# do-mpc/do-mpc

Measured on AMD Instinct MI355X. Metric: MPC steps/sec (make_step wall-time), industrial_poly robust multi-stage, higher is better.
Workload: dtype f64

## Files before the change

__graft_entry__.py:

```python
import os
import subprocess
import sys

ROOT = os.path.dirname(os.path.abspath(__file__))
if ROOT not in sys.path:
    sys.path.insert(0, ROOT)

PREBUILT = [
    ("oscillating_masses", {}),
    ("batch_reactor", {}),
    ("batch_reactor", {"n_horizon": 50}),
    ("CSTR", {}),
    ("CSTR", {"n_robust": 0, "collocation_deg": 3}),
    ("CSTR", {"track_sign": -3000.0}),
    ("industrial_poly", {}),
    ("industrial_poly", {"n_robust": 2, "uncertainty": "paired"}),
    ("industrial_poly", {"collocation_deg": 3, "collocation_ni": 2, "n_horizon": 6}),
    ("kinematic_bicycle", {}),
    ("dynamic_bicycle", {}),
    ("kite", {"n_horizon": 20}),
    ("rotating_masses", {}),
    ("CSTR", {"custom_rterm": "default_as_expression"}),
    ("CSTR", {"custom_rterm": "custom"}),
    ("oscillating_masses", {"custom_rterm": "custom"}),
    ("oscillating_masses_dae", {}),
    ("dip", {}),
    ("CSTR", {"n_robust": 0, "nl_cons_check_colloc_points": True}),
    ("dip", {"n_horizon": 40, "nl_cons_check_colloc_points": True}),
    ("CSTR", {"nl_cons_single_slack": True}),
    ("CSTR", {"nl_cons_single_slack": True, "n_robust": 2, "n_horizon": 8, "uncertainty": {"alpha": [1.0, 1.05, 0.95], "beta": [1.0]}}),
    ("CSTR", {"nl_cons_single_slack": True, "n_robust": 0, "nl_cons_check_colloc_points": True}),
    ("CSTR", {"open_loop": True, "uncertainty": {"alpha": [1.0, 1.05, 0.95], "beta": [1.0]}}),
    ("CSTR", {"open_loop": True, "n_robust": 2, "n_horizon": 6, "uncertainty": {"alpha": [1.0, 1.05], "beta": [1.0]}, "soft_T_R": False}),
    ("shape_family:s1", {}), ("shape_family:s2", {}), ("shape_family:s3", {}), ("shape_family:s4", {}), ("shape_family:s5", {}),
    ("shape_family:s6", {}), ("shape_family:s7", {}), ("shape_family:s8", {}), ("shape_family:s9", {}),
]

PREBUILT_BATCH = [
    ("industrial_poly", {}), ("industrial_poly", {"n_robust": 2, "uncertainty": "paired"}),
    ("oscillating_masses", {}), ("CSTR", {}), ("CSTR", {"n_robust": 0, "collocation_deg": 3}), ("batch_reactor", {}), ("batch_reactor", {"n_horizon": 50}),
    ("rotating_masses", {}),
]
PREBUILT_BATCH_MHE = [("rotating_masses", "build_mhe", {}, {}), ("rotating_masses", "build_mhe_w", {"process_noise": True}, {}),
                      ("rotating_masses", "build_mhe_w", {"process_noise": True}, {"scaling": "MHE_W_SCALING"})]


PREBUILT_DEFS = [("CSTR", {}, "DOMPC_FORCE_DENSE=1"), ("batch_reactor", {}, "DOMPC_FORCE_DENSE=1"),
                 ("CSTR", {}, "DOMPC_GJ_U=1e9"), ("industrial_poly", {}, "DOMPC_GJ_U=1e9"),
                 ("batch_reactor", {}, "DOMPC_REG_GJ=0"), ("batch_reactor", {}, "DOMPC_GJ_U=1e9"),
                 ("industrial_poly", {}, "DOMPC_QUAD=0"), ("CSTR", {}, "DOMPC_QUAD=0"), ("CSTR", {"n_horizon": 5, "n_robust": 0}, "DOMPC_QUAD=0")]

PREBUILT_NODE_PACK = [("industrial_poly", {}), ("CSTR", {})] + [("shape_family:s%d" % i, {}) for i in range(1, 10)]
PREBUILT_BATCH_FAMILY = [("shape_family:s%d" % i, {}) for i in range(1, 10)]

PREBUILT_QUAD_LDS = [("DOMPC_QUAD_LDS=1", [("industrial_poly", {}), ("CSTR", {})]),
                     ("DOMPC_GJ_U=1e9", [("industrial_poly", {})]),
                     ("DOMPC_GJ_U=1e9 DOMPC_QUAD_LDS=1", [("industrial_poly", {})])]

PREBUILT_FWD_STAGE = [("DOMPC_FWD_STAGE=0", [("industrial_poly", {}), ("CSTR", {})]),
                      ("DOMPC_GJ_U=1e9 DOMPC_FWD_STAGE=0", [("industrial_poly", {})])]

PREBUILT_MO_READS = [("DOMPC_MO_BRANCHED=1", [("industrial_poly", {}), ("CSTR", {})]),
                     ("DOMPC_GJ_U=1e9 DOMPC_MO_BRANCHED=1", [("industrial_poly", {})])]

PREBUILT_SHARD = [
    ("CSTR", {}),
    ("industrial_poly", {"n_robust": 2, "uncertainty": "paired"}),
]


PREBUILT_MHE = [("rotating_masses", "build_mhe", {}, {}), ("rotating_masses", "build_mhe_w", {"process_noise": True}, {}),
                ("rotating_masses", "build_mhe_w", {"process_noise": True}, {"scaling": "MHE_W_SCALING"}),
                ("rotating_masses", "build_mhe", {"dae": True}, {}), ("rotating_masses", "build_mhe_w", {"process_noise": True, "dae": True}, {}),
                ("oscillating_masses", "build_mhe", {"estimation": True}, {}), ("oscillating_masses", "build_mhe", {"estimation": True, "dae": True}, {}),
                ("rotating_masses", "build_mhe_w", {"process_noise": True}, {"soft_limit": (-0.1, 0.01)}),
                ("rotating_masses", "build_mhe_w", {"process_noise": True}, {"soft_limit": (-0.1, 0.01), "nl_cons_single_slack": True}),
                ("rotating_masses", "build_mhe_w", {"process_noise": True, "input_meas_noise": False}, {})]


PREBUILT_ROUTE = [("oscillating_masses", "docstring", False, False), ("oscillating_masses", "tree", False, False),
                  ("industrial_poly", "tree", False, True), ("CSTR", "tree", False, True), ("batch_reactor", "tree", False, False),
                  ("oscillating_masses_dae", "tree", False, False), ("rotating_masses", "tree", False, False),
                  ("CSTR", "docstring", False, False), ("batch_reactor", "docstring", False, False), ("industrial_poly", "docstring", False, False),
                  ("oscillating_masses", None, True, False), ("CSTR", None, True, False), ("CSTR", "tree", True, False),
                  ("industrial_poly", None, True, False), ("industrial_poly", "tree", True, False), ("batch_reactor", None, True, False),
                  ("rotating_masses", None, True, False)]


def lowered_route_cases():
    from do_mpc_amd import controller
    from do_mpc_amd.examples import CASES
    tests = os.path.join(ROOT, "tests")
    if tests not in sys.path:
        sys.path.insert(0, tests)
    import route_cases as rc
    out = []
    orig = controller.HipIpmSolver
    controller.HipIpmSolver = _NoSolver
    try:
        for name, cost, rows, batch in PREBUILT_ROUTE:
            ex = CASES[name]
            mpc = rc.stopped_before_setup(lambda n: ex.build_mpc(ex.build_model()), name)
            mpc.prepare_nlp()
            if rows:
                rc.rows_at_three_nodes(mpc, name)
            if cost:
                rc.ADDED_COST[cost](mpc)
            mpc.create_nlp()
            out.append((f"{name} + {cost or ''}{' + rows' if rows else ''} (low-level route)", {}, mpc.generated_header, mpc.model_hash, batch))
    finally:
        controller.HipIpmSolver = orig
    return out


PREBUILT_PLANTS = ["oscillating_masses", "batch_reactor", "CSTR", "industrial_poly", "oscillating_masses_dae", "dip", "rotating_masses",
                   "triple_tank", "batch_reactor_lqr_dae", "batch_reactor_lqr_dae:build_dae_model", "cstr_lqr", "oscillating_masses_lqr"]

PREBUILT_PLANT_FAMILY = ["ode", "dae", "discrete"]


def lowered_plant_family(entries=None):
    from do_mpc_amd.simulator import Simulator
    tests = os.path.join(ROOT, "tests")
    if tests not in sys.path:
        sys.path.insert(0, tests)
    import plant_family_common as pf
    out = []
    for kind in (PREBUILT_PLANT_FAMILY if entries is None else entries):
        hdr = Simulator(pf.build_model(kind))._lower()
        out.append((kind, hdr, hdr.rsplit('PLANT_MODEL_HASH "', 1)[1].split('"')[0]))
    return out


PREBUILT_EKF = [("triple_tank", {}), ("oscillating_masses", {"estimation": True}), ("rotating_masses", {}), ("CSTR", {})]


def lowered_ekf(entries=None):
    from do_mpc_amd.ekf import EKF
    from do_mpc_amd.examples import CASES
    out = []
    for name, kw in (PREBUILT_EKF if entries is None else entries):
        hdr = EKF(CASES[name].build_model(**kw))._lower()
        out.append((name, kw, hdr, hdr.rsplit('EKF_MODEL_HASH "', 1)[1].split('"')[0]))
    return out


PREBUILT_EKF_DAE = ["masses", "nonlinear_discrete", "continuous", "dip", "batch_reactor", "limit", "status", "oscillating_masses_dae",
# ... 92 lines not shown
        if plant.startswith("family:"):
            (_, ph, p_hash), = lowered_plant_family([plant.split(":", 1)[1]])
        else:
            case, _, builder = plant.partition(":")
            ph = Simulator(getattr(CASES[case], builder or "build_model")())._lower()
            p_hash = ph.rsplit('PLANT_MODEL_HASH "', 1)[1].split('"')[0]
        (net_label, nh, n_hash), = lowered_ampc([shape])
        out.append((f"{plant} x {net_label}", ph, nh, p_hash, n_hash))
    return out


PREBUILT_ASMPC = [(1, 1), (4, 1), (4, 2), (17, 3), (3, 16), (64, 16)]


def lowered_asmpc(entries=None):
    from do_mpc_amd import lowering
    out = []
    for nx, nu in (PREBUILT_ASMPC if entries is None else entries):
        hdr = lowering.lower_asmpc(nx, nu)
        out.append((f"n_x = {nx}, n_u = {nu}", hdr, hdr.rsplit('ASMPC_MODEL_HASH "', 1)[1].split('"')[0]))
    return out


class _NoSolver:

    def __init__(self, *a, **k):
        pass


def lowered_models(which=None):
    from do_mpc_amd import controller
    from do_mpc_amd.examples import CASES
    out = []
    orig = controller.HipIpmSolver
    controller.HipIpmSolver = _NoSolver
    try:
        for name, kw in (PREBUILT if which is None else which):
            ex = CASES[name]
            mpc = ex.build_mpc(ex.build_model(), **kw)
            out.append((name, kw, mpc.generated_header, mpc.model_hash))
        if which is None:
            out += _lower_mhe(PREBUILT_MHE)
    finally:
        controller.HipIpmSolver = orig
    return out


def _lower_mhe(entries):
    from do_mpc_amd.examples import CASES
    out = []
    for name, builder, mkw, bkw in entries:
        ex = CASES[name]
        bkw = {k: (getattr(ex, v) if isinstance(v, str) else v) for k, v in bkw.items()}
        mhe = getattr(ex, builder)(ex.build_model(**mkw), **bkw)
        out.append((f"{name} ({builder})", {**mkw, **{k: "..." for k in bkw}}, mhe._mpc.generated_header, mhe._mpc.model_hash))
    return out


def lowered_mhe(entries):
    from do_mpc_amd import controller
    orig = controller.HipIpmSolver
    controller.HipIpmSolver = _NoSolver
    try:
        return _lower_mhe(entries)
    finally:
        controller.HipIpmSolver = orig


def build() -> None:
    from do_mpc_amd import build as nb
    import do_mpc_amd
    from concurrent.futures import ThreadPoolExecutor
    lib = nb.runtime_library()
    print("[build] runtime:", lib, flush=True)
    jobs = [(f"{name} {kw}", header, h, False, False, "") for name, kw, header, h in lowered_models()]
    jobs += [(f"{name} {kw}", header, h, True, False, "") for name, kw, header, h in lowered_models(PREBUILT_SHARD)]
    jobs += [(f"{name} {kw}", header, h, False, True, "") for name, kw, header, h in lowered_models(PREBUILT_BATCH + PREBUILT_BATCH_FAMILY)]
    jobs += [(f"{name} {kw}", header, h, False, True, "") for name, kw, header, h in lowered_mhe(PREBUILT_BATCH_MHE)]
    route = lowered_route_cases()
    jobs += [(f"{name} {kw}", header, h, False, False, "") for name, kw, header, h, _ in route]
    jobs += [(f"{name} {kw}", header, h, False, True, "") for name, kw, header, h, batch in route if batch]
    for name, kw, defs in PREBUILT_DEFS:
        jobs += [(f"{name} {kw}", header, h, False, False, defs) for _, _, header, h in lowered_models([(name, kw)])]
    for defs, classes in [("DOMPC_NODE_PACK=0", PREBUILT_NODE_PACK)] + PREBUILT_QUAD_LDS + PREBUILT_FWD_STAGE + PREBUILT_MO_READS:
        jobs += [(f"{name} {kw}", header, h, False, batch, defs) for name, kw, header, h in lowered_models(classes) for batch in (False, True)]
    with ThreadPoolExecutor(max_workers=max(1, min(len(jobs), (os.cpu_count() or 2) - 1))) as pool:
        outs = list(pool.map(lambda j: nb.model_code_object(j[1], j[2], shard=j[3], batch_only=j[4], defs=j[5]), jobs))
    for (label, _, _, shard, batch, defs), co in zip(jobs, outs):
        print(f"[build] {label}{' [' + defs + ']' if defs else ''}{' (tree sharding)' if shard else ''}{' (batch only)' if batch else ''}: {co}", flush=True)
    from do_mpc_amd.examples import CASES
    from do_mpc_amd.simulator import Simulator
    for name in PREBUILT_PLANTS:
        case, _, builder = name.partition(":")
        hdr = Simulator(getattr(CASES[case], builder or "build_model")())._lower()
        co = nb.plant_code_object(hdr, hdr.rsplit('PLANT_MODEL_HASH "', 1)[1].split('"')[0])
        print(f"[build] plant {name}: {co}")
    for kind, hdr, h in lowered_plant_family():
        print(f"[build] plant of the probe family '{kind}': {nb.plant_code_object(hdr, h)}")
    failed = []
    for entry in PREBUILT_EKF:
        try:
            for name, kw, hdr, h in lowered_ekf([entry]):
                print(f"[build] filter {name} {kw}: {nb.ekf_code_object(hdr, h)}")
        except Exception as e:
            failed.append(entry)
            print(f"[build] filter {entry[0]} {entry[1]}: FAILED\n{e}")
    for entry in PREBUILT_EKF_DAE:
        try:
            for name, hdr, h in lowered_ekf_dae([entry]):
                print(f"[build] filter of a model with algebraic states '{name}': {nb.ekf_code_object(hdr, h)}")
        except Exception as e:
            failed.append(entry)
            print(f"[build] filter of a model with algebraic states '{entry}': FAILED\n{e}")
    failed_lqr = []
    for entry in PREBUILT_LQR:
        try:
            for label, hdr, h in lowered_lqr([entry]):
                print(f"[build] LQR design {label}: {nb.lqr_code_object(hdr, h)}")
        except Exception as e:
            failed_lqr.append(entry)
            print(f"[build] LQR design {entry}: FAILED\n{e}")
    failed_ampc = []
    for entry in PREBUILT_AMPC:
        try:
            for label, hdr, h in lowered_ampc([entry]):
                print(f"[build] approximate MPC network {label}: {nb.ampc_code_object(hdr, h)}")
        except Exception as e:
            failed_ampc.append(entry)
            print(f"[build] approximate MPC network {entry}: FAILED\n{e}")
    failed_ampc_loop = []
    for entry in PREBUILT_AMPC_LOOP:
        try:
            for label, ph, nh, p_hash, n_hash in lowered_ampc_loop([entry]):
                co = nb.ampc_loop_code_object(ph, nh, nb.ampc_loop_pair_hash(p_hash, n_hash))
                print(f"[build] approximate MPC loop {label}: {co}")
                if entry[1] not in PREBUILT_AMPC:
                    print(f"[build] approximate MPC network of that pair: {nb.ampc_code_object(nh, n_hash)}")
        except Exception as e:
            failed_ampc_loop.append(entry)
            print(f"[build] approximate MPC loop {entry}: FAILED\n{e}")
    failed_asmpc = []
    for entry in PREBUILT_ASMPC:
        try:
            for label, hdr, h in lowered_asmpc([entry]):
                print(f"[build] sensitivity-based MPC law {label}: {nb.asmpc_code_object(hdr, h)}")
        except Exception as e:
            failed_asmpc.append(entry)
            print(f"[build] sensitivity-based MPC law {entry}: FAILED\n{e}")
    mk = os.path.join(ROOT, "oracle", "Makefile")
    if os.path.exists(mk):
        subprocess.run(["make", "-C", os.path.join(ROOT, "oracle")], check=True)
    if failed:
        raise RuntimeError(f"extended Kalman filter code objects that could not be built: {failed}")
    if failed_lqr:
        raise RuntimeError(f"LQR design code objects that could not be built: {failed_lqr}")
    if failed_ampc:
        raise RuntimeError(f"approximate MPC code objects that could not be built: {failed_ampc}")
    if failed_ampc_loop:
        raise RuntimeError(f"approximate MPC loop code objects that could not be built: {failed_ampc_loop}")
    if failed_asmpc:
        raise RuntimeError(f"sensitivity-based MPC law code objects that could not be built: {failed_asmpc}")


def smoke() -> None:
    import numpy as np
    from do_mpc_amd.examples import CASES
    from oracle import ipm
# ... 64 lines not shown
```

do_mpc_amd/csrc/dompc_kernel.h:

```cpp
#pragma once
#include <math.h>
#include <stdint.h>
#include "dompc_kargs.h"
#include "dompc_lanes.h"

namespace dompc {

#ifndef DOMPC_HOST_EMU
#define DOMPC_PHASE __device__ inline
#else
#define DOMPC_PHASE static inline
#endif

constexpr int NX = DOMPC_NX, NU = DOMPC_NU, NP = DOMPC_NP, NTVP = DOMPC_NTVP;
#ifndef DOMPC_EPS_GLOBAL
#define DOMPC_EPS_GLOBAL 0
#endif
constexpr bool EPS_GLOBAL = DOMPC_EPS_GLOBAL != 0 && DOMPC_NS > 0 && DOMPC_NE > 0;
constexpr int NS = EPS_GLOBAL ? 0 : DOMPC_NS;
constexpr int NSE = DOMPC_NS;
constexpr int NVG_MAX = 32;
constexpr int NZ = DOMPC_NZ;
constexpr int DEG = DOMPC_DEG, NI = DOMPC_NI, M = DOMPC_M;
#ifndef DOMPC_NL_COLLOC
#define DOMPC_NL_COLLOC 0
#endif
#ifndef DOMPC_FREE_ROOT
#define DOMPC_FREE_ROOT 0
#endif
#ifndef DOMPC_LT_END
#define DOMPC_LT_END 0
#endif
#ifndef DOMPC_NL_DUP
#define DOMPC_NL_DUP 0
#endif
#if !DOMPC_FREE_ROOT
DOMPC_FN double dompc_aterm_f(const double*, const double*, const double*, const double*) { return 0.0; }
DOMPC_FN void dompc_aterm(const double*, const double*, const double*, const double*, double*, double*, double*) {}
#endif
constexpr bool FREE_ROOT = DOMPC_FREE_ROOT != 0, LT_END = DOMPC_LT_END != 0 && M > 0;
constexpr int NEB = DOMPC_NE;
constexpr int NLP = (DOMPC_NL_COLLOC && M > 0) ? M : 1;
constexpr bool NL_DUP = DOMPC_NL_DUP != 0 && NEB > 0;
constexpr int NLB = NLP + (NL_DUP ? 1 : 0);
constexpr int NE = NEB * NLB;
constexpr bool NL_COLLOC = DOMPC_NL_COLLOC && M > 0 && NEB > 0;
DOMPC_HD constexpr int nl_pt(int blk) { return blk < NLP ? blk : NLP - 1; }
#ifndef DOMPC_FORCE_DENSE
#define DOMPC_FORCE_DENSE 0
#endif
constexpr bool DENSE_EDGE = DOMPC_NZ > 0 || NL_COLLOC || NL_DUP || LT_END || DOMPC_FORCE_DENSE;
DOMPC_HD inline int nl_slack(int i) { return DOMPC_NL_SLACK[NLB == 1 ? i : i % NEB]; }
constexpr int NA = NX + NU;
constexpr int NV = NU + NS;
constexpr int NYT = NA + NV;
constexpr int MZ = NZ > 0 ? (M > 0 ? M : 1) : 0;
constexpr int NWX = M * NX;
constexpr int NW = NWX + MZ * NZ;
constexpr bool RT_CUSTOM = DOMPC_RTERM_CUSTOM != 0;
constexpr int NR = NA + NU, NR_T = NR * (NR + 1) / 2;
constexpr int RT_LEN = RT_CUSTOM ? 1 + NR + NR_T : 0;
constexpr int NF = NX + NZ;
constexpr int NAV = NA + NZ;
constexpr int NCOLL = NI * DEG;
constexpr int RPE = NW + NX + NE;
constexpr int NE1 = NE > 0 ? NE : 1, NEB1 = NEB > 0 ? NEB : 1;
constexpr int NS1 = NS > 0 ? NS : 1;
constexpr int NW1 = NW > 0 ? NW : 1;
constexpr int MAX_FILTER = 48;
#ifndef DOMPC_SHARD
#define DOMPC_SHARD 0
#endif
#ifndef DOMPC_GJ_U
#define DOMPC_GJ_U 0.01
#endif
constexpr int RED_MAX = 12;
#ifndef DOMPC_HOST_EMU
constexpr int GS_C = 64;
#else
constexpr int GS_C = 1;
#endif

constexpr int LU_N = (NI == 1 && DEG > 0 && !DENSE_EDGE) ? DEG * NX : NW;
constexpr int EW_LU = 0;
constexpr int EW_SIGW = EW_LU + LU_N * LU_N;
constexpr int EW_RW = EW_SIGW + NW;
constexpr int EW_JD = EW_RW + NW;
// ... 611 lines not shown
```

do_mpc_amd/csrc/dompc_quad.h:

```cpp
#if !defined(DOMPC_HOST_EMU) && DOMPC_DEG >= 1 && DOMPC_M >= 1 && DOMPC_NI == 1 && DOMPC_NX + DOMPC_NU + 2 <= 16 && DOMPC_DEG * DOMPC_DEG * DOMPC_NX <= 64

using dompc_lanes::rbc;
using dompc_lanes::pin;
using dompc_lanes::fmac_rbc;
using dompc_lanes::dpp_ready;
using dompc_lanes::sfor;

struct MoRef { int kind, off; };
constexpr MoRef moref_in(int d, const int* vidx, int nv, const int* cidx, int nc, int base) {
  for (int k = 0; k < nv; ++k) if (vidx[k] == d) return MoRef{2, base + k};
  for (int k = 0; k < nc; ++k) if (cidx[k] == d) return MoRef{1, k};
  return MoRef{0, 0};
}
constexpr MoRef moref_dyn(int p, int d) { return moref_in(d, DOMPC_DYN_VIDX, DOMPC_DYN_NV, DOMPC_DYN_CIDX, DOMPC_DYN_NC, p * DOMPC_DYN_NV); }
constexpr MoRef moref_lt(int d) { return moref_in(d, DOMPC_LT_VIDX, DOMPC_LT_NV, DOMPC_LT_CIDX, DOMPC_LT_NC, MOC_LT); }
constexpr MoRef moref_nl(int d) { return moref_in(d, DOMPC_NL_VIDX, DOMPC_NL_NV, DOMPC_NL_CIDX, DOMPC_NL_NC, MOC_NL); }
constexpr MoRef moref_mt(int d) { return moref_in(d, DOMPC_MT_VIDX, DOMPC_MT_NV, DOMPC_MT_CIDX, DOMPC_MT_NC, MOC_MT); }
#ifndef DOMPC_MO_BRANCHED
#define DOMPC_MO_BRANCHED 0
#endif
#define MO_BR_SWEEP (DOMPC_MO_BRANCHED == 1 || DOMPC_MO_BRANCHED == 2)
#define MO_BR_FWD (DOMPC_MO_BRANCHED == 1 || DOMPC_MO_BRANCHED == 3)
template <bool BRANCHED>
struct MoRec {
  const ldsd* p;
  __device__ inline double at(int off) const {
    if constexpr (BRANCHED) return p[off];
    else return ((const volatile ldsd*)p)[off];
  }
};
template <int KIND, int OFF, class REC>
__device__ inline double mo_dyn_val(REC rec) { if constexpr (KIND == 2) return rec.at(OFF); else if constexpr (KIND == 1) return DOMPC_DYN_CVAL[OFF]; else return 0.0; }
template <int KIND, int OFF, class REC>
__device__ inline double mo_lt_val(REC rec) { if constexpr (KIND == 2) return rec.at(OFF); else if constexpr (KIND == 1) return DOMPC_LT_CVAL[OFF]; else return 0.0; }
template <int KIND, int OFF, class REC>
__device__ inline double mo_nl_val(REC rec) { if constexpr (KIND == 2) return rec.at(OFF); else if constexpr (KIND == 1) return DOMPC_NL_CVAL[OFF]; else return 0.0; }
template <int KIND, int OFF, class REC>
__device__ inline double mo_mt_val(REC rec) { if constexpr (KIND == 2) return rec.at(OFF); else if constexpr (KIND == 1) return DOMPC_MT_CVAL[OFF]; else return 0.0; }
constexpr bool qd_f_linear() {
  for (int i = 0; i < NX; ++i) if (DOMPC_DYN_VIDX[i] != i) return false;
  return true;
}

struct QdPack { int woff, row0, xoffp, xoffc, level, epsoff; double om; };
__device__ inline QdPack qd_pack(const KArgs& A, int e, double sf) {
  const auto* ep = A.edge_pack + e * EP_N;
  QdPack k;
  k.woff = ep[EP_WOFF]; k.row0 = ep[EP_ROW0]; k.xoffp = ep[EP_XOFF_PARENT]; k.xoffc = ep[EP_XOFF_CHILD]; k.level = ep[EP_LEVEL]; k.epsoff = ep[EP_EPSOFF_PARENT];
  k.om = __builtin_bit_cast(double, ((unsigned long long)(unsigned)ep[EP_OMEGA_HI] << 32) | (unsigned long long)(unsigned)ep[EP_OMEGA_LO]) * sf;
  return k;
}
__device__ inline void stage_quad(const Prob& Q, int e0, int lane, ldsd* Ld, int bank) {
  const double* src = Q.mo + (int64_t)e0 * MO_REC;
  ldsd* dst = Ld + bank * QL_MOSZ;
#pragma unroll
  for (int q = 0; q < QL_MOSZ / 128; ++q)
    __builtin_amdgcn_global_load_lds((const __attribute__((address_space(1))) void*)(src + 128 * q + 2 * lane),
                                     (__attribute__((address_space(3))) void*)(dst + 128 * q), 16, 0, 0);
}

#ifndef DOMPC_QUAD_PROFILE
#define DOMPC_QUAD_PROFILE DOMPC_PROFILE
#endif
#ifndef DOMPC_QUAD_LDS
#define DOMPC_QUAD_LDS 0
#endif
#define QD_SB() __builtin_amdgcn_sched_barrier(0)

__device__ inline int eval_edge_quad(const Thr& T, const Prob& Q, int e0, int e0n, double mu, int lane_, ldsd* Ld, int bank, const QdPack& pk, QdPack& pkn, bool store_lu) {
  const KArgs& A = *Q.A;
  int lane = lane_;
  asm volatile("" : "+v"(lane));
  constexpr int R = DEG * NX;
  constexpr double GJ_U = DOMPC_GJ_U;
  const int g = lane >> 4, j = lane & 15;
  const bool act = e0 + g < A.n_edges;
  const int e = act ? e0 + g : A.n_edges - 1;
  const bool isx = j < NX;
  const bool st_x = act && isx;
  const unsigned b = (unsigned)(isx ? j : 0);
  const bool soc = (Q.soc & 1) != 0;
  const double omh = (Q.soc & 2) ? 0.0 : pk.om;
#if DOMPC_QUAD_PROFILE
  long long pc0 = prof_clock();
#define QD_PH(i) if (T.prof && T.tid == 0) { const long long pc1 = prof_clock(); T.prof[i] += pc1 - pc0; pc0 = pc1; }
#else
#define QD_PH(i)
#endif
  const double xn = ldoff(Q.x, (unsigned)pk.xoffp + b), xc = ldoff(Q.x, (unsigned)pk.xoffc + b);
// ... 74 lines not shown
  for (int s = 0; s < M; ++s) { pin(BGv[s]); pin(BBv[s]); pin(SGv[s]); pin(ZDv[s]); }
#pragma unroll
  for (int jj = 0; jj < DEG; ++jj) pin(res[jj]);
  pin(rc); pin(ce);
  double bc[DEG][R];
  sfor<DEG>([&](auto S_) {
    constexpr int s = S_;
    sfor<R>([&](auto R_) {
      constexpr int r = R_, jj = r / NX, a = r % NX;
      double v = 0.0;
      if constexpr (s == jj)
        sfor<NX>([&](auto B_) {
          constexpr int bb = B_;
          constexpr MoRef rf = moref_dyn(jj, NX + a * NA + bb);
          if constexpr (rf.kind != 0) { const double t_ = mo_dyn_val<rf.kind, rf.off>(rec); v = (j == bb) ? t_ : v; }
        });
      if constexpr (s == 0) {
        sfor<NU>([&](auto K_) {
          constexpr int ku = K_;
          constexpr MoRef rf = moref_dyn(jj, NX + a * NA + NX + ku);
          if constexpr (rf.kind != 0) { const double t_ = mo_dyn_val<rf.kind, rf.off>(rec); v = (j == NX + ku) ? t_ : v; }
        });
        const double rb_ = rbc<a>(res[jj]);
        v = (j == NA) ? rb_ : v;
      }
      v = (j == a) ? v - DOMPC_C[(s + 1) * (DEG + 1) + jj + 1] : v;
      bc[s][r] = v;
    });
  });
  QD_PH(5)
  QD_SB();
  double RWv[M], RDv[M], ry;
  {
    double tcol[M];
#pragma unroll
    for (int s = 0; s < M; ++s) tcol[s] = 0.0;
    double ryu = 0.0;
    sfor<DEG>([&](auto J_) {
      constexpr int jj = J_;
      sfor<NX>([&](auto A_) {
        constexpr int a = A_;
        const double la = rbc<a>(lam[jj]);
        tcol[jj] = fma(la, bc[jj][jj * NX + a], tcol[jj]);
        if constexpr (jj == 0) ryu = fma(la, bc[0][a], ryu);
        else ryu = fma(la, bc[0][jj * NX + a], ryu);
      });
    });
#pragma unroll
    for (int s = 0; s < DEG; ++s) {
      double t = tcol[s];
#pragma unroll
      for (int jj = 0; jj < DEG; ++jj)
        if (jj != s) t = fma(-DOMPC_C[(s + 1) * (DEG + 1) + jj + 1], lam[jj], t);
      tcol[s] = t - DOMPC_D[s + 1] * lamc;
    }
    tcol[M - 1] = lamc + nue;
    double ryx = -DOMPC_D[0] * lamc;
#pragma unroll
    for (int jj = 0; jj < DEG; ++jj) ryx = fma(-DOMPC_C[0 * (DEG + 1) + jj + 1], lam[jj], ryx);
    ry = isx ? ryx : ryu;
#pragma unroll
    for (int s = 0; s < M; ++s) { RWv[s] = tcol[s] + BGv[s]; RDv[s] = tcol[s] + ZDv[s]; }
#pragma unroll
    for (int s = 0; s < M; ++s) { pin(RWv[s]); pin(RDv[s]); }
    pin(ry);
    if (isx) {
      ldsd* Lv = Ld + QL_RW + g * QL_VG;
#pragma unroll
      for (int s = 0; s < M; ++s) { Lv[s * NX + (int)b] = RWv[s]; Lv[NW + s * NX + (int)b] = BBv[s]; }
    }
  }
  QD_PH(6)
  QD_SB();
  int bad = 0;
  double sig[DEG];
#pragma unroll
  for (int s = 0; s < DEG; ++s) sig[s] = 1.0;
  sfor<R>([&](auto K_) {
    constexpr int k = K_, sk = k / NX, bk = k % NX;
    constexpr int rt1 = (4 * (k / 4 + 1) < R) ? 4 * (k / 4 + 1) : R;
    QD_SB();
    const bool own = (j == bk);
    double m = 0.0;
#pragma unroll
    for (int r = k + 1; r < rt1; ++r) m = fmax(m, fabs(bc[sk][r]));
    const double akk = fabs(bc[sk][k]);
    bad |= (int)(own & !(akk >= GJ_U * m && akk > 1e-300));
    const double pl = fast_rcp((akk > 1e-300) ? bc[sk][k] : 1.0);
    const double pinv = rbc<bk>(pl);
    sig[sk] = own ? -pl : sig[sk];
    double pm[DEG];
#pragma unroll
    for (int s = 0; s < DEG; ++s) {
      const double prow = bc[s][k] * pinv;
      pm[s] = (s == sk && own) ? 0.0 : -prow;
      bc[s][k] = (s == sk && own) ? -1.0 : prow;
      pin(pm[s]);
    }
    asm volatile("s_nop 1");
    sfor<R>([&](auto R_) {
      constexpr int r = R_;
      if constexpr (r != k) {
        sfor<DEG>([&](auto S_) { constexpr int s = S_; if constexpr (s != sk) fmac_rbc<bk>(bc[s][r], bc[sk][r], pm[s]); });
        fmac_rbc<bk>(bc[sk][r], bc[sk][r], pm[sk]);
      }
    });
#pragma unroll
    for (int s = 0; s < DEG; ++s)
#pragma unroll
      for (int r = 0; r < R; ++r) pin(bc[s][r]);
  });
  QD_SB();
#pragma unroll
  for (int s = 0; s < DEG; ++s)
#pragma unroll
    for (int r = 0; r < R; ++r) bc[s][r] *= sig[s];
  QD_SB();
  if (__ballot(bad) != 0ull) return 2;
  QD_PH(2)
  QD_SB();
  if (st_x) {
    if (!soc) {
#pragma unroll
      for (int jj = 0; jj < DEG; ++jj) Q.c[pk.row0 + jj * NX + (int)b] = res[jj];
      Q.c[pk.row0 + R + (int)b] = rc;
      Q.c[pk.row0 + NW + (int)b] = ce;
    }
#pragma unroll
    for (int s = 0; s < M; ++s) {
      const int gi = pk.woff + s * NX + (int)b;
      Q.rd[gi] = RDv[s];
    }
    double* ew = Q.ew + (int64_t)e * EW_SIZE;
    if (store_lu) {
#pragma unroll
      for (int s = 0; s < DEG; ++s)
#pragma unroll
        for (int r = 0; r < R; ++r) ew[EW_LU + r * LU_N + s * NX + (int)b] = bc[s][r];
    }
#pragma unroll
    for (int s = 0; s < M; ++s) {
      ew[EW_SIGW + s * NX + (int)b] = SGv[s] + Q.dsw;
      ew[EW_RW + s * NX + (int)b] = RWv[s];
    }
  }
  if (e0n >= 0) stage_quad(Q, e0n, lane, Ld, bank ^ 1);
  {
    const int en = (e0n >= 0 ? e0n : e0) + g;
    pkn = qd_pack(A, en < A.n_edges ? en : A.n_edges - 1, Q.sf);
  }
  double Wc[NW];
  {
#pragma unroll
    for (int r = 0; r < R; ++r) {
      double t = (isx ? DOMPC_C[0 * (DEG + 1) + 1] : -1.0) * bc[0][r];
#pragma unroll
      for (int s = 1; s < DEG; ++s) t = fma(isx ? DOMPC_C[0 * (DEG + 1) + s + 1] : 0.0, bc[s][r], t);
      Wc[r] = t;
    }
    sfor<NX>([&](auto A_) {
      constexpr int a = A_;
      const double rcb = rbc<a>(rc);
      double t = (j == NA) ? -rcb : ((j == a) ? DOMPC_D[0] : 0.0);
#pragma unroll
      for (int s = 1; s <= DEG; ++s) t = fma(DOMPC_D[s], Wc[(s - 1) * NX + a], t);
      Wc[R + a] = t;
    });
  }
#pragma unroll
  for (int r = 0; r < NW; ++r) pin(Wc[r]);
  double* S_ = Q.es + (int64_t)e * ES_SIZE;
  {
    double cv = 0.0;
    sfor<NX>([&](auto A_) {
      constexpr int a = A_;
      if (act && j < NA) S_[ES_AB + a * NA + j] = Wc[R + a];
      const double w0a = rbc<NA>(Wc[R + a]);
      cv = (j == a) ? w0a + ce : cv;
    });
    pin(cv);
    if (st_x) S_[ES_CV + (int)b] = cv;
  }
  QD_PH(7)
  QD_SB();
  double acc[NA];
// ... 276 lines not shown
  mu = ufl(mu);
  const int ng = T.nt / 64, gid = group_index(T.tid, 64), lane = T.tid % 64;
  ldsd* Ld = T.edge_lds + (int64_t)(T.ltid / 64) * EL_SIZE;
  const int nq = (A.n_edges + 3) / 4;
  int fail = 0, bank = 0;
  int qd = gid;
  if (qd >= nq) return 0;
  const bool store_lu = lu_store_rule(A, mu, Q.soc);
  const int gl = lane >> 4;
  auto pack_of = [&](int q) { const int e = 4 * q + gl; return qd_pack(A, e < A.n_edges ? e : A.n_edges - 1, Q.sf); };
  stage_quad(Q, 4 * qd, lane, Ld, 0);
  QdPack pk = pack_of(qd);
  while (qd < nq) {
    const int qn = qd + ng;
    const bool more = qn < nq;
    QdPack pkn = pk;
    const int rc = eval_edge_quad(T, Q, 4 * qd, more ? 4 * qn : -1, mu, lane, Ld, bank, pk, pkn, store_lu);
    if (__builtin_amdgcn_readfirstlane(rc) == 2) {
      pkn = pack_of(more ? qn : qd);
      asm volatile("s_waitcnt vmcnt(0)" ::: "memory");
      fail |= phase_edge_fallback(kp, Q.slot, b_, 4 * qd, Q.soc, Q.sf, mu, Q.dsw);
      if (more) stage_quad(Q, 4 * qn, lane, Ld, bank ^ 1);
    } else {
      fail |= rc;
    }
    bank ^= 1;
    pk = pkn;
    qd = qn;
  }
  return fail;
}
__device__ inline int sweep_quads(const Thr& T, const Prob& Q, double mu) {
  const KArgs& A = *Q.A;
  const int b_ = (int)((Q.P - A.p) / A.n_opt_p);
  return phase_sweep_quads(T.kp, b_, Q.slot, Q.soc, Q.sf, mu, Q.dsw);
}
#elif !defined(DOMPC_HOST_EMU)
__device__ inline int sweep_quads(const Thr&, const Prob&, double) { return 0; }
#endif

#if !defined(DOMPC_HOST_EMU) && DOMPC_DEG >= 1 && DOMPC_M >= 1 && DOMPC_NI == 1 && DOMPC_NX + DOMPC_NU + 2 <= 16 && DOMPC_DEG * DOMPC_DEG * DOMPC_NX <= 64
static_assert(!QUAD_FWD || (2 * NW + NA + DEG * NX <= QF_VG && QL_WB + 4 * QF_VG <= EL_SIZE), "LDS of the four-edge forward pass");

__device__ inline void qd_fw_columns(MoRec<MO_BR_FWD> rec, int j, const double (&res)[DEG], double (&bc)[DEG][DEG * NX]) {
  constexpr int R = DEG * NX;
  sfor<DEG>([&](auto S_) {
    constexpr int s = S_;
    sfor<R>([&](auto R_) {
      constexpr int r = R_, jj = r / NX, a = r % NX;
      double v = 0.0;
      if constexpr (s == jj)
        sfor<NX>([&](auto B_) {
          constexpr int bb = B_;
          constexpr MoRef rf = moref_dyn(jj, NX + a * NA + bb);
          if constexpr (rf.kind != 0) { const double t_ = mo_dyn_val<rf.kind, rf.off>(rec); v = (j == bb) ? t_ : v; }
        });
      if constexpr (s == 0) {
        sfor<NU>([&](auto K_) {
          constexpr int ku = K_;
          constexpr MoRef rf = moref_dyn(jj, NX + a * NA + NX + ku);
          if constexpr (rf.kind != 0) { const double t_ = mo_dyn_val<rf.kind, rf.off>(rec); v = (j == NX + ku) ? t_ : v; }
        });
        const double rb_ = rbc<a>(res[jj]);
        v = (j == NA) ? rb_ : v;
      }
      v = (j == a) ? v - DOMPC_C[(s + 1) * (DEG + 1) + jj + 1] : v;
      bc[s][r] = v;
    });
  });
}
__device__ inline int qd_fw_eliminate(int j, double (&bc)[DEG][DEG * NX]) {
  constexpr int R = DEG * NX;
  constexpr double GJ_U = DOMPC_GJ_U;
  int bad = 0;
  double sig[DEG];
#pragma unroll
  for (int s = 0; s < DEG; ++s) sig[s] = 1.0;
  sfor<R>([&](auto K_) {
    constexpr int k = K_, sk = k / NX, bk = k % NX;
    constexpr int rt1 = (4 * (k / 4 + 1) < R) ? 4 * (k / 4 + 1) : R;
    QD_SB();
    const bool own = (j == bk);
    double m = 0.0;
#pragma unroll
    for (int r = k + 1; r < rt1; ++r) m = fmax(m, fabs(bc[sk][r]));
    const double akk = fabs(bc[sk][k]);
    bad |= (int)(own & !(akk >= GJ_U * m && akk > 1e-300));
    const double pl = fast_rcp((akk > 1e-300) ? bc[sk][k] : 1.0);
    const double pinv = rbc<bk>(pl);
    sig[sk] = own ? -pl : sig[sk];
    double pm[DEG];
#pragma unroll
    for (int s = 0; s < DEG; ++s) {
      const double prow = bc[s][k] * pinv;
      pm[s] = (s == sk && own) ? 0.0 : -prow;
      bc[s][k] = (s == sk && own) ? -1.0 : prow;
      pin(pm[s]);
    }
    asm volatile("s_nop 1");
    sfor<R>([&](auto R_) {
      constexpr int r = R_;
      if constexpr (r != k) {
        sfor<DEG>([&](auto S_) { constexpr int s = S_; if constexpr (s != sk) fmac_rbc<bk>(bc[s][r], bc[sk][r], pm[s]); });
        fmac_rbc<bk>(bc[sk][r], bc[sk][r], pm[sk]);
      }
    });
#pragma unroll
    for (int s = 0; s < DEG; ++s)
#pragma unroll
      for (int r = 0; r < R; ++r) pin(bc[s][r]);
  });
  QD_SB();
#pragma unroll
  for (int s = 0; s < DEG; ++s)
#pragma unroll
    for (int r = 0; r < R; ++r) bc[s][r] *= sig[s];
  QD_SB();
  return bad;
}

struct QfPack { int woff, row0, level, n, cn, uoffp, epsoff; };
__device__ inline QfPack qf_pack(const KArgs& A, int e) {
  const auto* ep = A.edge_pack + e * EP_N;
  QfPack k;
  k.woff = ep[EP_WOFF]; k.row0 = ep[EP_ROW0]; k.level = ep[EP_LEVEL]; k.n = ep[EP_PARENT]; k.cn = ep[EP_CHILD];
  k.uoffp = ep[EP_UOFF_PARENT]; k.epsoff = ep[EP_EPSOFF_PARENT];
  return k;
}

constexpr bool QF_STAGED = QF_STAGE && EW_SIGW % 2 == 0;
static_assert(EP_N == 16, "one index record per row of 16 lanes");
__device__ inline int qf_index_request(const KArgs& A, int e0, int lane) {
  const int e = min(e0 + (lane >> 4), A.n_edges - 1);
  return A.edge_pack[(int64_t)e * EP_N + (lane & 15)];
}
template <int F>
__device__ inline int qf_row_field(int ipk) { return __builtin_amdgcn_update_dpp(0, ipk, 0x150 + F, 0xf, 0xf, true); }
__device__ inline void qf_glds4(const double* src, int word, ldsd* dst) {
  __builtin_amdgcn_global_load_lds((const __attribute__((address_space(1))) void*)((const unsigned*)src + word),
                                   (__attribute__((address_space(3))) void*)dst, 4, 0, 0);
}
__device__ inline void stage_quad_operands(const Prob& Q, int e0, int ipk, int lane, ldsd* Ld) {
  const KArgs& A = *Q.A;
  ldsd* dst = Ld + QF_SG;
  static_assert(EW_RW == EW_SIGW + NW, "Sigma_w | r_w is one run of 2 NW doubles");
  static_assert(!QF_STAGED || (EW_SIGW % 2 == 0 && EW_SIZE % 8 == 0 && QF_SG % 2 == 0), "16-byte pieces of Sigma_w | r_w, in memory and in LDS");
#pragma unroll
  for (int p = 0; p < 2; ++p) {
    const int e = min(e0 + 2 * p + (lane >> 5), A.n_edges - 1);
    const double* src = Q.ew + (int64_t)e * EW_SIZE + EW_SIGW + 2 * min(lane & 31, NW - 1);
    __builtin_amdgcn_global_load_lds((const __attribute__((address_space(1))) void*)src,
                                     (__attribute__((address_space(3))) void*)(dst + QF_SG_EW + 128 * p), 16, 0, 0);
  }
  const int k = min(lane >> 1, 2 * NX + NU - 1), h = lane & 1;
  sfor<4>([&](auto G_) {
    constexpr int gg = G_;
    const int row0 = __builtin_amdgcn_readlane(ipk, 16 * gg + EP_ROW0), n = __builtin_amdgcn_readlane(ipk, 16 * gg + EP_PARENT);
    qf_glds4(Q.c + row0, min(lane, 2 * NW - 1), dst + QF_SG_C + 32 * gg);
    const double* xs = Q.nd + (int64_t)n * ND_SIZE + ND_DXT + k;
    const double* ns = Q.dlam + row0 + NW + (k - NX);
    const double* vs = k < NX ? xs : ns;
    if constexpr (NU > 0) {
      const int uoffp = __builtin_amdgcn_readlane(ipk, 16 * gg + EP_UOFF_PARENT);
      const double* us = Q.dx + uoffp + (k - 2 * NX);
      vs = k < 2 * NX ? vs : us;
    }
    qf_glds4(vs, h, dst + QF_SG_V + 32 * gg);
  });
}

__device__ __attribute__((noinline)) void phase_forward_quads(const void* kp, int b_, int slot, int soc, double sf, double delta_, int cl_) {
  const KArgs A = kernel_args(kp);
  Thr T = make_thr(A);
  T.kp = kp;
  Prob Q = make_prob(A, ufl(slot), A.p + (int64_t)ufl(b_) * A.n_opt_p);
  Q.sf = ufl(sf);
  Q.soc = ufl(soc);
  prob_bounds(Q);
  const double delta = ufl(delta_);
  const int cl = ufl(cl_);
  (void)delta;
  constexpr int R = DEG * NX;
  const int ng = T.nt / 64, gid = group_index(T.tid, 64);
  ldsd* Ld = T.edge_lds + (int64_t)(T.ltid / 64) * EL_SIZE;
  const int nq = (A.n_edges + 3) / 4;
  int bank = 0;
  int qd = gid;
  if (qd >= nq) return;
  {
    const int lane0 = (int)(threadIdx.x & 63u);
    stage_quad(Q, 4 * qd, lane0, Ld, 0);
  }
  int ipk = 0, ipkn = 0;
  if constexpr (QF_STAGED) {
    const int lane0 = (int)(threadIdx.x & 63u);
    ipk = qf_index_request(A, 4 * qd, lane0);
    stage_quad_operands(Q, 4 * qd, ipk, lane0, Ld);
  }
#if DOMPC_QUAD_PROFILE
  long long pc0 = prof_clock();
#define QF_PH(i) if (T.prof && T.tid == 0) { const long long pc1 = prof_clock(); T.prof[i] += pc1 - pc0; pc0 = pc1; }
#else
#define QF_PH(i)
#endif
  while (qd < nq) {
    int lane = (int)(threadIdx.x & 63u);
    asm volatile("" : "+v"(lane));
    const int g = lane >> 4, j = lane & 15;
    const int e0 = 4 * qd;
    const bool act = e0 + g < A.n_edges;
    const int e = act ? e0 + g : A.n_edges - 1;
    const bool isx = j < NX, st_x = act && isx;
    const int b = isx ? j : 0;
    QfPack pk;
    if constexpr (QF_STAGED) {
      pk.woff = qf_row_field<EP_WOFF>(ipk); pk.row0 = qf_row_field<EP_ROW0>(ipk); pk.level = qf_row_field<EP_LEVEL>(ipk);
      pk.n = 0; pk.cn = qf_row_field<EP_CHILD>(ipk); pk.uoffp = 0; pk.epsoff = qf_row_field<EP_EPSOFF_PARENT>(ipk);
    } else {
      pk = qf_pack(A, e);
    }
    const bool chain = pk.level >= cl;
    double dxn, ccont, dnu;
    double du[NU > 0 ? NU : 1];
    double cres[DEG], rwv[M], sgv[M];
    const double* ew = Q.ew + (int64_t)e * EW_SIZE;
    if constexpr (!QF_STAGED) {
      dxn = Q.nd[(int64_t)pk.n * ND_SIZE + ND_DXT + b];
#pragma unroll
      for (int u = 0; u < NU; ++u) du[u] = Q.dx[pk.uoffp + u];
#pragma unroll
      for (int jj = 0; jj < DEG; ++jj) cres[jj] = Q.c[pk.row0 + jj * NX + b];
      ccont = Q.c[pk.row0 + R + b];
#pragma unroll
      for (int s = 0; s < M; ++s) { rwv[s] = ew[EW_RW + s * NX + b]; sgv[s] = ew[EW_SIGW + s * NX + b]; }
      dnu = Q.dlam[pk.row0 + NW + b];
    } else {
      dnu = 0.0;
    }
    if (__ballot(!chain) != 0ull) {
      const double* Nc = Q.nd + (int64_t)pk.cn * ND_SIZE;
      double t = Nc[ND_PV + b];
#pragma unroll
      for (int bb = 0; bb < NA; ++bb) t = fma(Nc[ND_P + b * NA + bb], Nc[ND_DXT + bb], t);
      dnu = chain ? dnu : t;
    }
    if constexpr (!QF_STAGED) { QF_PH(17) }
    asm volatile("s_waitcnt vmcnt(0)" ::: "memory");
    __builtin_amdgcn_fence(__ATOMIC_ACQ_REL, "wavefront");
    __builtin_amdgcn_wave_barrier();
    QF_PH(15)
    if constexpr (QF_STAGED) {
      if (qd + ng < nq) ipkn = qf_index_request(A, 4 * (qd + ng), lane);
      const ldsd* So = Ld + QF_SG;
      dxn = So[QF_SG_V + 32 * g + b];
      const double dnus = So[QF_SG_V + 32 * g + NX + b];
      dnu = chain ? dnus : dnu;
#pragma unroll
      for (int u = 0; u < NU; ++u) du[u] = So[QF_SG_V + 32 * g + 2 * NX + u];
#pragma unroll
      for (int jj = 0; jj < DEG; ++jj) cres[jj] = So[QF_SG_C + 32 * g + jj * NX + b];
      ccont = So[QF_SG_C + 32 * g + R + b];
#pragma unroll
      for (int s = 0; s < M; ++s) { rwv[s] = So[QF_SG_EW + 64 * g + NW + s * NX + b]; sgv[s] = So[QF_SG_EW + 64 * g + s * NX + b]; }
    }
    const MoRec<MO_BR_FWD> rec{Ld + bank * QL_MOSZ + (e - e0) * MO_REC};
    ldsd* Lv = Ld + QL_WB + g * QF_VG;
    constexpr int V_DW = 0, V_DY = NW, V_RHS = NW + NA, V_RR = 2 * NW + NA;
#if MO_BR_FWD
    if (isx) Lv[V_DY + j] = dxn;
    sfor<NU>([&](auto U_) { constexpr int u = U_; if (j == NX + u) Lv[V_DY + NX + u] = du[u]; });
#else
    {
      double dyv = dxn;
      sfor<NU>([&](auto U_) { constexpr int u = U_; dyv = (j == NX + u) ? du[u] : dyv; });
      if (j < NA) Lv[V_DY + j] = dyv;
    }
#endif
    double gv[DEG];
    sfor<DEG>([&](auto J_) {
      constexpr int jj = J_;
      double t = cres[jj] - DOMPC_C[0 * (DEG + 1) + jj + 1] * dxn;
      sfor<NX>([&](auto A_) {
        constexpr int a = A_;
        sfor<NU>([&](auto U_) {
          constexpr int u = U_;
          constexpr MoRef rf = moref_dyn(jj, NX + a * NA + NX + u);
          if constexpr (rf.kind != 0) { const double t_ = mo_dyn_val<rf.kind, rf.off>(rec) * du[u]; t += (j == a) ? t_ : 0.0; }
        });
      });
      gv[jj] = t;
      pin(gv[jj]);
    });
    QD_SB();
    double bc[DEG][R];
    qd_fw_columns(rec, j, gv, bc);
    QF_PH(28)
    QD_SB();
    const int bad = qd_fw_eliminate(j, bc);
    const bool fb = __ballot(bad) != 0ull;
    QF_PH(29)
    const int qn = qd + ng;
    if (qn < nq) stage_quad(Q, 4 * qn, lane, Ld, bank ^ 1);
    if constexpr (QF_STAGED) {
      if (qn < nq) {
        asm volatile("s_waitcnt lgkmcnt(0)" ::: "memory");
        stage_quad_operands(Q, 4 * qn, ipkn, lane, Ld);
      }
      QF_PH(17)
    }
    double dwv[M];
    if (!fb) {
#pragma unroll
      for (int s = 0; s < DEG; ++s) dwv[s] = 0.0;
      sfor<R>([&](auto R_) {
        constexpr int r = R_, s = r / NX, a = r % NX;
        const double t_ = rbc<NA>(bc[0][r]);
        dwv[s] = (j == a) ? -t_ : dwv[s];
      });
    } else {
      __builtin_amdgcn_fence(__ATOMIC_ACQ_REL, "wavefront");
      __builtin_amdgcn_wave_barrier();
      if (isx) {
#pragma unroll
        for (int s = 0; s < DEG; ++s) Lv[V_RR + s * NX + j] = gv[s];
      }
      __builtin_amdgcn_fence(__ATOMIC_ACQ_REL, "wavefront");
      __builtin_amdgcn_wave_barrier();
#pragma unroll
      for (int s = 0; s < DEG; ++s) {
        double t = 0.0;
        for (int k2 = 0; k2 < R; ++k2) t -= ew[EW_LU + (s * NX + b) * LU_N + k2] * Lv[V_RR + k2];
        dwv[s] = t;
      }
      __builtin_amdgcn_fence(__ATOMIC_ACQ_REL, "wavefront");
      __builtin_amdgcn_wave_barrier();
    }
    {
      double t = DOMPC_D[0] * dxn - ccont;
#pragma unroll
      for (int s = 1; s <= DEG; ++s) t = fma(DOMPC_D[s], dwv[s - 1], t);
      dwv[M - 1] = t;
    }
    if (isx) {
#pragma unroll
      for (int s = 0; s < M; ++s) Lv[V_DW + s * NX + j] = dwv[s];
    }
    __builtin_amdgcn_fence(__ATOMIC_ACQ_REL, "wavefront");
    __builtin_amdgcn_wave_barrier();
    QF_PH(30)
    QD_SB();
    double rhs[M];
    sfor<M>([&](auto S_) {
      constexpr int s = S_;
      double t = fma(sgv[s], dwv[s], rwv[s]);
      if constexpr (s == M - 1) t += dnu;
      if constexpr (s < DEG) {
        sfor<NA>([&](auto I_) {
          constexpr int i = I_;
          sfor<NA - i>([&](auto D_) {
            constexpr int k = i + D_;
            constexpr MoRef rf = moref_dyn(s, MOH_H0 + symi(i, k, NA));
            if constexpr (rf.kind != 0 && i < NX) {
              const double h = mo_dyn_val<rf.kind, rf.off>(rec);
              if constexpr (k < NX) {
                const double pk_ = h * (double)Lv[V_DW + s * NX + k];
                t += (j == i) ? pk_ : 0.0;
                if constexpr (i != k) { const double pi_ = h * (double)Lv[V_DW + s * NX + i]; t += (j == k) ? pi_ : 0.0; }
              } else {
                const double pu_ = h * du[k - NX];
                t += (j == i) ? pu_ : 0.0;
              }
            }
          });
        });
      }
      rhs[s] = -t;
      pin(rhs[s]);
    });
    QF_PH(31)
    QD_SB();
    if (isx) {
#pragma unroll
      for (int s = 0; s < DEG; ++s) Lv[V_RR + s * NX + j] = fma(DOMPC_D[s + 1], rhs[M - 1], rhs[s]);
    }
    __builtin_amdgcn_fence(__ATOMIC_ACQ_REL, "wavefront");
    __builtin_amdgcn_wave_barrier();
    double dl[M];
    if (!fb) {
#pragma unroll
// ... 46 lines not shown
```

Baseline: 11120.

## Skip structurally-zero Gauss-Jordan updates and issue forward-quad index reads early

Adds a compile-time sparsity table built from the model's dynamics Jacobian pattern with symbolic fill-in, and uses it to drop pivot-search comparisons and elimination FMAs on row pairs that stay zero in the collocation Gauss-Jordan solve. Separately, the forward-quad loop now reads the index fields into scalar registers before staging the quad data, so the operand addresses are known earlier and the loads can overlap. Both are on by default and can be turned off with defines. The skip relies on the structural zeros matching the real numeric values, and the early request adds an extra index fetch on the last iteration.

```diff
diff --git a/__graft_entry__.py b/__graft_entry__.py
--- a/__graft_entry__.py
+++ b/__graft_entry__.py
@@ -63,6 +63,9 @@
 PREBUILT_MO_READS = [("DOMPC_MO_BRANCHED=1", [("industrial_poly", {}), ("CSTR", {})]),
                      ("DOMPC_GJ_U=1e9 DOMPC_MO_BRANCHED=1", [("industrial_poly", {})])]
 
+PREBUILT_GJ_SKIP = [("DOMPC_GJ_SKIP=0 DOMPC_FWD_REQ_EARLY=0", [("industrial_poly", {}), ("CSTR", {})]),
+                    ("DOMPC_GJ_U=1e9 DOMPC_GJ_SKIP=0 DOMPC_FWD_REQ_EARLY=0", [("industrial_poly", {})])]
+
 PREBUILT_SHARD = [
     ("CSTR", {}),
     ("industrial_poly", {"n_robust": 2, "uncertainty": "paired"}),
@@ -321,7 +324,7 @@
     jobs += [(f"{name} {kw}", header, h, False, True, "") for name, kw, header, h, batch in route if batch]
     for name, kw, defs in PREBUILT_DEFS:
         jobs += [(f"{name} {kw}", header, h, False, False, defs) for _, _, header, h in lowered_models([(name, kw)])]
-    for defs, classes in [("DOMPC_NODE_PACK=0", PREBUILT_NODE_PACK)] + PREBUILT_QUAD_LDS + PREBUILT_FWD_STAGE + PREBUILT_MO_READS:
+    for defs, classes in [("DOMPC_NODE_PACK=0", PREBUILT_NODE_PACK)] + PREBUILT_QUAD_LDS + PREBUILT_FWD_STAGE + PREBUILT_MO_READS + PREBUILT_GJ_SKIP:
         jobs += [(f"{name} {kw}", header, h, False, batch, defs) for name, kw, header, h in lowered_models(classes) for batch in (False, True)]
     with ThreadPoolExecutor(max_workers=max(1, min(len(jobs), (os.cpu_count() or 2) - 1))) as pool:
         outs = list(pool.map(lambda j: nb.model_code_object(j[1], j[2], shard=j[3], batch_only=j[4], defs=j[5]), jobs))
diff --git a/do_mpc_amd/csrc/dompc_gj_structure.h b/do_mpc_amd/csrc/dompc_gj_structure.h
--- /dev/null
+++ b/do_mpc_amd/csrc/dompc_gj_structure.h
@@ -0,0 +1,78 @@
+#pragma once
+#include <stdint.h>
+
+#ifndef DOMPC_GJ_SKIP
+#define DOMPC_GJ_SKIP 1
+#endif
+
+namespace dompc_gj {
+
+constexpr int NX = DOMPC_NX, NU = DOMPC_NU, DEG = DOMPC_DEG, NA = NX + NU;
+constexpr int R = DEG * NX;
+constexpr int NCOL = R + NU + 1;
+#ifdef DOMPC_NZ
+constexpr int NZ_ = DOMPC_NZ;
+#else
+constexpr int NZ_ = 0;
+#endif
+constexpr bool USABLE = DOMPC_DEG >= 1 && DOMPC_NI == 1 && NZ_ == 0 && NCOL <= 64;
+constexpr int RD = USABLE ? R : 1;
+
+constexpr bool jac_present(int a, int b) {
+  const int d = NX + a * NA + b;
+  for (int k = 0; k < DOMPC_DYN_NV; ++k) if (DOMPC_DYN_VIDX[k] == d) return true;
+  for (int k = 0; k < DOMPC_DYN_NC; ++k) if (DOMPC_DYN_CIDX[k] == d) return true;
+  return false;
+}
+
+struct Table {
+  bool skip[RD][RD];
+  int n_skip;
+};
+
+constexpr Table make_table(bool use_model) {
+  Table t{};
+  if (!USABLE) return t;
+  uint64_t pat[RD] = {};
+  for (int r = 0; r < R; ++r) {
+    const int jj = r / NX, a = r % NX;
+    uint64_t m = 0;
+    for (int c = 0; c < R; ++c) {
+      const int s = c / NX, b = c % NX;
+      if (a == b || (s == jj && (!use_model || jac_present(a, b)))) m |= uint64_t(1) << c;
+    }
+    for (int c = R; c < NCOL; ++c) m |= uint64_t(1) << c;
+    pat[r] = m;
+  }
+  for (int k = 0; k < R; ++k)
+    for (int r = 0; r < R; ++r) {
+      if (r == k) continue;
+      if (pat[r] >> k & 1) pat[r] |= pat[k];
+      else { t.skip[k][r] = true; ++t.n_skip; }
+    }
+  return t;
+}
+
+constexpr Table TABLE = make_table(true);
+constexpr Table TABLE_BLOCKS = make_table(false);
+constexpr int BLOCK_PAIRS = USABLE ? (DEG - 1) * (NX * (NX - 1) / 2) : 0;
+
+constexpr bool gj_skip(int k, int r) {
+  return DOMPC_GJ_SKIP != 0 && USABLE && k >= 0 && r >= 0 && k < R && r < R && TABLE.skip[k][r];
+}
+
+constexpr bool diagonal_kept() {
+  for (int k = 0; k < RD; ++k) if (TABLE.skip[k][k]) return false;
+  return true;
+}
+constexpr bool covers_blocks() {
+  for (int k = 0; k < RD; ++k)
+    for (int r = 0; r < RD; ++r) if (TABLE_BLOCKS.skip[k][r] && !TABLE.skip[k][r]) return false;
+  return true;
+}
+static_assert(diagonal_kept(), "nothing is skipped at r == k");
+static_assert(TABLE_BLOCKS.n_skip >= BLOCK_PAIRS && TABLE.n_skip >= TABLE_BLOCKS.n_skip && covers_blocks(),
+              "the table covers at least the pairs the block structure gives");
+static_assert(USABLE || TABLE.n_skip == 0, "a model without usable tables: nothing is skipped");
+
+}
diff --git a/do_mpc_amd/csrc/dompc_kernel.h b/do_mpc_amd/csrc/dompc_kernel.h
--- a/do_mpc_amd/csrc/dompc_kernel.h
+++ b/do_mpc_amd/csrc/dompc_kernel.h
@@ -3,6 +3,7 @@
 #include <stdint.h>
 #include "dompc_kargs.h"
 #include "dompc_lanes.h"
+#include "dompc_gj_structure.h"
 
 namespace dompc {
 
diff --git a/do_mpc_amd/csrc/dompc_quad.h b/do_mpc_amd/csrc/dompc_quad.h
--- a/do_mpc_amd/csrc/dompc_quad.h
+++ b/do_mpc_amd/csrc/dompc_quad.h
@@ -5,6 +5,7 @@
 using dompc_lanes::fmac_rbc;
 using dompc_lanes::dpp_ready;
 using dompc_lanes::sfor;
+using dompc_gj::gj_skip;
 
 struct MoRef { int kind, off; };
 constexpr MoRef moref_in(int d, const int* vidx, int nv, const int* cidx, int nc, int base) {
@@ -245,8 +246,10 @@
     QD_SB();
     const bool own = (j == bk);
     double m = 0.0;
-#pragma unroll
-    for (int r = k + 1; r < rt1; ++r) m = fmax(m, fabs(bc[sk][r]));
+    sfor<rt1 - k - 1>([&](auto D_) {
+      constexpr int r = k + 1 + D_;
+      if constexpr (!gj_skip(k, r)) m = fmax(m, fabs(bc[sk][r]));
+    });
     const double akk = fabs(bc[sk][k]);
     bad |= (int)(own & !(akk >= GJ_U * m && akk > 1e-300));
     const double pl = fast_rcp((akk > 1e-300) ? bc[sk][k] : 1.0);
@@ -263,7 +266,7 @@
     asm volatile("s_nop 1");
     sfor<R>([&](auto R_) {
       constexpr int r = R_;
-      if constexpr (r != k) {
+      if constexpr (r != k && !gj_skip(k, r)) {
         sfor<DEG>([&](auto S_) { constexpr int s = S_; if constexpr (s != sk) fmac_rbc<bk>(bc[s][r], bc[sk][r], pm[s]); });
         fmac_rbc<bk>(bc[sk][r], bc[sk][r], pm[sk]);
       }
@@ -706,8 +709,10 @@
     QD_SB();
     const bool own = (j == bk);
     double m = 0.0;
-#pragma unroll
-    for (int r = k + 1; r < rt1; ++r) m = fmax(m, fabs(bc[sk][r]));
+    sfor<rt1 - k - 1>([&](auto D_) {
+      constexpr int r = k + 1 + D_;
+      if constexpr (!gj_skip(k, r)) m = fmax(m, fabs(bc[sk][r]));
+    });
     const double akk = fabs(bc[sk][k]);
     bad |= (int)(own & !(akk >= GJ_U * m && akk > 1e-300));
     const double pl = fast_rcp((akk > 1e-300) ? bc[sk][k] : 1.0);
@@ -724,7 +729,7 @@
     asm volatile("s_nop 1");
     sfor<R>([&](auto R_) {
       constexpr int r = R_;
-      if constexpr (r != k) {
+      if constexpr (r != k && !gj_skip(k, r)) {
         sfor<DEG>([&](auto S_) { constexpr int s = S_; if constexpr (s != sk) fmac_rbc<bk>(bc[s][r], bc[sk][r], pm[s]); });
         fmac_rbc<bk>(bc[sk][r], bc[sk][r], pm[sk]);
       }
@@ -764,7 +769,23 @@
   __builtin_amdgcn_global_load_lds((const __attribute__((address_space(1))) void*)((const unsigned*)src + word),
                                    (__attribute__((address_space(3))) void*)dst, 4, 0, 0);
 }
-__device__ inline void stage_quad_operands(const Prob& Q, int e0, int ipk, int lane, ldsd* Ld) {
+#ifndef DOMPC_FWD_REQ_EARLY
+#define DOMPC_FWD_REQ_EARLY 1
+#endif
+struct QfReq { int row0[4], n[4], uoffp[4]; };
+__device__ inline QfReq qf_request_fields(int ipk) {
+  QfReq q;
+  sfor<4>([&](auto G_) {
+    constexpr int gg = G_;
+    q.row0[gg] = __builtin_amdgcn_readlane(ipk, 16 * gg + EP_ROW0);
+    q.n[gg] = __builtin_amdgcn_readlane(ipk, 16 * gg + EP_PARENT);
+    q.uoffp[gg] = NU > 0 ? __builtin_amdgcn_readlane(ipk, 16 * gg + EP_UOFF_PARENT) : 0;
+    asm volatile("" : "+s"(q.row0[gg]), "+s"(q.n[gg]), "+s"(q.uoffp[gg]));
+  });
+  return q;
+}
+template <class FIELD>
+__device__ inline void stage_quad_operands_of(const Prob& Q, int e0, FIELD field, int lane, ldsd* Ld) {
   const KArgs& A = *Q.A;
   ldsd* dst = Ld + QF_SG;
   static_assert(EW_RW == EW_SIGW + NW, "Sigma_w | r_w is one run of 2 NW doubles");
@@ -779,18 +800,24 @@
   const int k = min(lane >> 1, 2 * NX + NU - 1), h = lane & 1;
   sfor<4>([&](auto G_) {
     constexpr int gg = G_;
-    const int row0 = __builtin_amdgcn_readlane(ipk, 16 * gg + EP_ROW0), n = __builtin_amdgcn_readlane(ipk, 16 * gg + EP_PARENT);
+    const int row0 = field(G_, EP_ROW0), n = field(G_, EP_PARENT);
     qf_glds4(Q.c + row0, min(lane, 2 * NW - 1), dst + QF_SG_C + 32 * gg);
     const double* xs = Q.nd + (int64_t)n * ND_SIZE + ND_DXT + k;
     const double* ns = Q.dlam + row0 + NW + (k - NX);
     const double* vs = k < NX ? xs : ns;
     if constexpr (NU > 0) {
-      const int uoffp = __builtin_amdgcn_readlane(ipk, 16 * gg + EP_UOFF_PARENT);
+      const int uoffp = field(G_, EP_UOFF_PARENT);
       const double* us = Q.dx + uoffp + (k - 2 * NX);
       vs = k < 2 * NX ? vs : us;
     }
     qf_glds4(vs, h, dst + QF_SG_V + 32 * gg);
   });
+}
+__device__ inline void stage_quad_operands(const Prob& Q, int e0, int ipk, int lane, ldsd* Ld) {
+  stage_quad_operands_of(Q, e0, [&](auto G_, int f) { constexpr int gg = G_; return __builtin_amdgcn_readlane(ipk, 16 * gg + f); }, lane, Ld);
+}
+__device__ inline void stage_quad_operands(const Prob& Q, int e0, const QfReq& rq, int lane, ldsd* Ld) {
+  stage_quad_operands_of(Q, e0, [&](auto G_, int f) { constexpr int gg = G_; return f == EP_ROW0 ? rq.row0[gg] : f == EP_PARENT ? rq.n[gg] : rq.uoffp[gg]; }, lane, Ld);
 }
 
 __device__ __attribute__((noinline)) void phase_forward_quads(const void* kp, int b_, int slot, int soc, double sf, double delta_, int cl_) {
@@ -811,15 +838,21 @@
   int bank = 0;
   int qd = gid;
   if (qd >= nq) return;
-  {
+  int ipk = 0, ipkn = 0;
+  constexpr bool REQ_EARLY = QF_STAGED && DOMPC_FWD_REQ_EARLY != 0;
+  if constexpr (REQ_EARLY) {
+    const int lane0 = (int)(threadIdx.x & 63u);
+    ipk = qf_index_request(A, 4 * qd, lane0);
+    const QfReq rq = qf_request_fields(ipk);
+    stage_quad(Q, 4 * qd, lane0, Ld, 0);
+    stage_quad_operands(Q, 4 * qd, rq, lane0, Ld);
+  } else {
     const int lane0 = (int)(threadIdx.x & 63u);
     stage_quad(Q, 4 * qd, lane0, Ld, 0);
-  }
-  int ipk = 0, ipkn = 0;
-  if constexpr (QF_STAGED) {
-    const int lane0 = (int)(threadIdx.x & 63u);
-    ipk = qf_index_request(A, 4 * qd, lane0);
-    stage_quad_operands(Q, 4 * qd, ipk, lane0, Ld);
+    if constexpr (QF_STAGED) {
+      ipk = qf_index_request(A, 4 * qd, lane0);
+      stage_quad_operands(Q, 4 * qd, ipk, lane0, Ld);
+    }
   }
 #if DOMPC_QUAD_PROFILE
   long long pc0 = prof_clock();
@@ -874,7 +907,7 @@
     __builtin_amdgcn_wave_barrier();
     QF_PH(15)
     if constexpr (QF_STAGED) {
-      if (qd + ng < nq) ipkn = qf_index_request(A, 4 * (qd + ng), lane);
+      if (REQ_EARLY || qd + ng < nq) ipkn = qf_index_request(A, 4 * (qd + ng), lane);
       const ldsd* So = Ld + QF_SG;
       dxn = So[QF_SG_V + 32 * g + b];
       const double dnus = So[QF_SG_V + 32 * g + NX + b];
@@ -924,11 +957,20 @@
     const bool fb = __ballot(bad) != 0ull;
     QF_PH(29)
     const int qn = qd + ng;
-    if (qn < nq) stage_quad(Q, 4 * qn, lane, Ld, bank ^ 1);
-    if constexpr (QF_STAGED) {
+    if constexpr (!QF_STAGED) {
+      if (qn < nq) stage_quad(Q, 4 * qn, lane, Ld, bank ^ 1);
+    } else {
       if (qn < nq) {
-        asm volatile("s_waitcnt lgkmcnt(0)" ::: "memory");
-        stage_quad_operands(Q, 4 * qn, ipkn, lane, Ld);
+        if constexpr (REQ_EARLY) {
+          const QfReq rqn = qf_request_fields(ipkn);
+          stage_quad(Q, 4 * qn, lane, Ld, bank ^ 1);
+          asm volatile("s_waitcnt lgkmcnt(0)" ::: "memory");
+          stage_quad_operands(Q, 4 * qn, rqn, lane, Ld);
+        } else {
+          stage_quad(Q, 4 * qn, lane, Ld, bank ^ 1);
+          asm volatile("s_waitcnt lgkmcnt(0)" ::: "memory");
+          stage_quad_operands(Q, 4 * qn, ipkn, lane, Ld);
+        }
       }
       QF_PH(17)
     }
```

Result: no change. 11190, median of 6 (+0.6%).
